# mohsenzakeri/Movi

Measured on AMD Instinct MI355X. Metric: PML query Gbases/s on regular-thresholds index, higher is better.
Workload: dtype u64

## Files before the change

movi_amd/csrc/movi_abi.hip:

```cpp
#include "../../include/movi_hip.h"
#include "movi_kernels.hpp"
#include "movi_expand_host.hpp"

#include <algorithm>
#include <cstdio>
#include <cstdlib>
#include <chrono>
#include <cstring>
#include <string>
#include <unordered_map>
#include <vector>

#include <dlfcn.h>
#include <fcntl.h>
#include <rccl/rccl.h>
#include <sys/mman.h>
#include <sys/stat.h>
#include <thread>
#include <unistd.h>

using namespace movi;

namespace {

// ... 743 lines not shown
}
constexpr size_t kTallyBytes = 2u * kTallySlots * sizeof(unsigned long long);
static hipError_t read_tally(const unsigned long long *d_tally, unsigned long long (&sum)[2], hipStream_t s) {
    std::vector<unsigned long long> h(2u * kTallySlots);
    hipError_t e = hipMemcpyAsync(h.data(), d_tally, kTallyBytes, hipMemcpyDeviceToHost, s);
    if (e == hipSuccess) e = hipStreamSynchronize(s);
    sum[0] = sum[1] = 0;
    if (e == hipSuccess) for (uint32_t i = 0; i < kTallySlots; ++i) { sum[0] += h[2 * i]; sum[1] += h[2 * i + 1]; }
    return e;
}
static void sample_no_ff(movi_index *ix, hipStream_t s) {
    if (ix->ahead_tallied) return;
    unsigned long long *d_tally = nullptr, h_tally[2] = {0, 0};
    hipError_t e = hipMalloc(&d_tally, kTallyBytes);
    if (e == hipSuccess) e = hipMemsetAsync(d_tally, 0, kTallyBytes, s);
    if (e == hipSuccess) e = tally_no_ff_share(ix->kmode, ix->dev, 16, d_tally, s);
    if (e == hipSuccess) e = read_tally(d_tally, h_tally, s);
    if (d_tally) (void)hipFree(d_tally);
    if (e != hipSuccess) { (void)hipGetLastError(); return; }
    ix->ahead_no_ff = h_tally[1] ? (double)h_tally[0] / (double)h_tally[1] : 0.0;
    ix->ahead_tallied = true;
}
static bool ahead_wanted(movi_index *ix) {
    const uint64_t bytes = ahead_rows_bytes(ix->desc.r);
    size_t free_b = 0, total_b = 0;
    if (hipMemGetInfo(&free_b, &total_b) != hipSuccess) { (void)hipGetLastError(); return false; }
    return bytes <= total_b / 4 && free_b > bytes + std::max<uint64_t>(2ull << 30, bytes / 2);
}
constexpr double kAheadCountRatio = 0.67;
static int build_ahead(movi_index *ix, hipStream_t s, bool by_itself) {
    HIP_TRY(hipMalloc(&ix->d_rows2, ahead_rows_bytes(ix->desc.r)));
    uint64_t tail = 0;
    unsigned long long *d_tally = nullptr, h_tally[2] = {0, 0};
    hipError_t e = hipMalloc(&d_tally, kTallyBytes);
    if (e == hipSuccess) e = hipMemsetAsync(d_tally, 0, kTallyBytes, s);
    if (e == hipSuccess) e = build_ahead_rows(ix->kmode, ix->dev, ix->d_rows2, &tail, s, d_tally);
    if (e == hipSuccess) e = read_tally(d_tally, h_tally, s);
    if (d_tally) (void)hipFree(d_tally);
    if (e != hipSuccess) { (void)hipFree(ix->d_rows2); ix->d_rows2 = nullptr; return fail_hip(e, "building the look-ahead rows"); }
    ix->dev.rows2 = ix->d_rows2;
    ix->dev.rows2_tail = tail;
    ix->dev.hints = ahead_rows_hinted(ix->desc.r) ? 1u : 0u;
    ix->ahead_no_ff = h_tally[1] ? (double)h_tally[0] / (double)h_tally[1] : 0.0;
    ix->ahead_tallied = true;
    ix->dev.rows2_count = (!by_itself || ix->ahead_no_ff >= kAheadCountRatio) ? 1u : 0u;
    return MOVI_OK;
}

constexpr uint64_t kDeepAutoRows = 48ull << 20;
static bool deep_eligible(const movi_index *ix) {
    return ix->kmode == MOVI_MODE_REGULAR_THRESHOLDS && deep_rows_eligible(ix->desc.r);
}
static int build_deep(movi_index *ix, hipStream_t s) {
    HIP_TRY(hipMalloc(&ix->d_rows3, deep_rows_bytes(ix->desc.r)));
    hipError_t e = build_deep_rows(ix->kmode, ix->dev, ix->d_rows3, s);
    if (e == hipSuccess) e = hipStreamSynchronize(s);
    if (e != hipSuccess) { (void)hipFree(ix->d_rows3); ix->d_rows3 = nullptr; return fail_hip(e, "building the deep rows"); }
    ix->dev.rows3 = ix->d_rows3;
    return MOVI_OK;
}

static bool ftab_eligible(const movi_index *ix) {
    return (ix->kmode == MOVI_MODE_REGULAR_THRESHOLDS || ix->kmode == MOVI_MODE_REGULAR) && ix->dev.sigma - ix->dev.sep == 4;
}
static int build_ftab_table(movi_index *ix, uint32_t K, hipStream_t s) {
    const size_t bytes = (size_t)16 << (2 * K);
    HIP_TRY(hipMalloc(&ix->d_ftab, bytes));
    hipError_t e = build_ftab(ix->kmode, ix->dev, K, ix->d_ftab, s);
    if (e == hipSuccess) e = hipStreamSynchronize(s);
    if (e != hipSuccess) { (void)hipFree(ix->d_ftab); ix->d_ftab = nullptr; return fail_hip(e, "building the count query's interval table"); }
    ix->dev.ftab = ix->d_ftab;
    ix->dev.ftab_k = K;
    return MOVI_OK;
}

static void ensure_pml_tables(movi_index *ix, hipStream_t s, bool from_prepare = false) {
    if (ix->kmer_auto > 0 && !ix->d_kmer && kmer_eligible(ix)) {
        if (build_kmer(ix, (uint32_t)ix->kmer_auto, s) != MOVI_OK) {
            (void)hipGetLastError();
            ix->kmer_auto = 0;
        }
    }
    if (ix->ahead_auto > 0 && !ix->d_rows2 && ahead_eligible(ix) && (from_prepare || !ix->prepared)) {
        if (ix->ahead_retry_in > 0) ix->ahead_retry_in -= 1;
        else if (!ahead_wanted(ix)) ix->ahead_retry_in = 63;
        else if (build_ahead(ix, s, true) != MOVI_OK) {
            (void)hipGetLastError();
            ix->ahead_auto = 0;
        }
    }
    if (ix->deep_auto > 0 && !ix->d_rows3 && deep_eligible(ix) && ix->desc.r <= kDeepAutoRows && (from_prepare || !ix->prepared)) {
        if (!ix->ahead_tallied) sample_no_ff(ix, s);
        size_t free_b = 0, total_b = 0;
        const uint64_t bytes = deep_rows_bytes(ix->desc.r);
        if (ix->ahead_tallied && ix->ahead_no_ff < kAheadCountRatio) {
            ix->deep_auto = 0;
        } else if (hipMemGetInfo(&free_b, &total_b) != hipSuccess || free_b < bytes + (2ull << 30) || build_deep(ix, s) != MOVI_OK) {
            (void)hipGetLastError();
            ix->deep_auto = 0;
        }
    }
}

extern "C" {

int movi_index_get_desc(const movi_index_t *ix, movi_index_desc_t *desc) {
    if (!ix || !desc) return fail(MOVI_ERR_ARG, "NULL argument");
    *desc = ix->desc;
    desc->id_blocks = nullptr;
    desc->separator_thresholds = nullptr;
    desc->separator_map = nullptr;
    desc->tally_ids = nullptr;
    return MOVI_OK;
}

int movi_index_device_rows(const movi_index_t *ix, const void **d_rows, size_t *bytes) {
    if (!ix || !d_rows || !bytes) return fail(MOVI_ERR_ARG, "NULL argument");
    *d_rows = ix->d_rows;
    *bytes = ix->kmode != (int)ix->desc.mode ? (size_t)ix->desc.r * 8 : ix->rows_bytes;
    return MOVI_OK;
}

int movi_set_option(movi_index_t *ix, const char *key, int64_t value) {
    if (!ix || !key) return fail(MOVI_ERR_ARG, "NULL argument");
    if (!strcmp(key, "pml_variant")) {
        if (value != -1 && value != 0 && value != 1 && value != 14)
            return fail(MOVI_ERR_ARG, "pml_variant must be -1 (auto), 0, 1 or 14");
        ix->cfg.pml_variant = (int)value;
        return MOVI_OK;
    }
    if (!strcmp(key, "zml_variant")) {
        if (value < -1 || value > 1) return fail(MOVI_ERR_ARG, "zml_variant must be -1 (auto), 0 or 1");
        ix->cfg.zml_variant = (int)value;
        return MOVI_OK;
    }
    if (!strcmp(key, "count_variant")) {
        if (value < -1 || value > 1) return fail(MOVI_ERR_ARG, "count_variant must be -1 (auto), 0 or 1");
        ix->cfg.count_variant = (int)value;
        return MOVI_OK;
    }
    if (!strcmp(key, "idx64")) {
        if (value != 0 && value != 1) return fail(MOVI_ERR_ARG, "idx64 must be 0 or 1");
        ix->dev.idx32 = (value == 0 && ix->desc.r < 0xFFFFFFFFull) ? 1u : 0u;
        return MOVI_OK;
    }
    if (!strcmp(key, "block_threads")) {
        if (value != 0 && value != 64 && value != 128 && value != 192 && value != 256)
// ... 303 lines not shown
}

int movi_pml_expand_device(movi_index_t *ix, const uint32_t *d_mask_words, const uint64_t *d_offsets, uint64_t n_reads,
                           uint64_t n_bases, uint64_t first_base, uint16_t *d_out_pml, void *stream) {
    if (!ix) return fail(MOVI_ERR_ARG, "index handle is NULL");
    if (n_reads == 0) return MOVI_OK;
    if (!d_mask_words || !d_offsets || (n_bases && !d_out_pml)) return fail(MOVI_ERR_ARG, "NULL device buffer");
    HIP_TRY(hipSetDevice(ix->device));
    HIP_TRY(launch_pml_expand(d_mask_words, d_offsets, n_reads, n_bases, (uint32_t)(first_base & 31u), d_out_pml,
                              static_cast<hipStream_t>(stream)));
    return MOVI_OK;
}

int movi_zml_device(movi_index_t *ix, const uint8_t *d_bases, const uint64_t *d_offsets, uint64_t n_reads,
                    uint64_t n_bases, uint16_t *d_out_zml, uint8_t *d_read_err, const uint32_t *d_read_order,
                    void *stream) {
    return ml_device(true, ix, d_bases, d_offsets, n_reads, n_bases, d_out_zml, d_read_err, d_read_order, stream);
}

int movi_last_launch(const movi_index_t *ix, movi_launch_info_t *info) {
    if (!ix || !info) return fail(MOVI_ERR_ARG, "NULL argument");
    memset(info, 0, sizeof(*info));
    static_assert(sizeof(info->kernel) == sizeof(ix->last_launch.kernel), "kernel name buffers differ");
    memcpy(info->kernel, ix->last_launch.kernel, sizeof(info->kernel));
    info->variant = ix->last_launch.variant;
    info->block_threads = ix->last_launch.block_threads;
    info->waves_per_cu = ix->last_launch.waves_per_cu;
    info->segmented = ix->last_launch.segmented;
    info->idx64 = ix->last_launch.idx64;
    info->staged = ix->last_launch.staged;
    info->ahead = ix->last_launch.ahead;
    return MOVI_OK;
}

int movi_launch_log(char *buf, size_t cap, size_t *needed) {
    const size_t n = take_launch_log(buf, cap);
    if (needed) *needed = n + 1;
    return MOVI_OK;
}

int movi_index_info(const movi_index_t *ix, const char *key, double *value) {
    if (!ix || !key || !value) return fail(MOVI_ERR_ARG, "NULL argument");
    const double rows = ix->kmode != (int)ix->desc.mode ? (double)ix->desc.r * 8.0 : (double)ix->rows_bytes;
    const double kmer = ix->d_kmer ? (double)((size_t)16 << (2 * ix->dev.kmer_k)) : 0.0;
    const double ftab = ix->d_ftab ? (double)((size_t)16 << (2 * ix->dev.ftab_k)) : 0.0;
    const double ahead = ix->d_rows2 ? (double)ahead_rows_bytes(ix->desc.r) : 0.0;
    const double deep = ix->d_rows3 ? (double)deep_rows_bytes(ix->desc.r) : 0.0;
    const double ckpt = ix->d_ckpt ? (double)((ix->desc.r >> kPrefixShift) + 2) * 8.0 : 0.0;
    if (!strcmp(key, "rows_bytes")) *value = rows;
    else if (!strcmp(key, "kmer_bytes")) *value = kmer;
    else if (!strcmp(key, "ftab_bytes")) *value = ftab;
    else if (!strcmp(key, "ahead_rows_bytes")) *value = ahead;
    else if (!strcmp(key, "deep_rows_bytes")) *value = deep;
    else if (!strcmp(key, "ckpt_bytes")) *value = ckpt;
    else if (!strcmp(key, "derived_bytes")) *value = kmer + ftab + ahead + deep + ckpt;
    else if (!strcmp(key, "ahead_no_ff")) *value = ix->ahead_tallied ? ix->ahead_no_ff : -1.0;
    else if (!strcmp(key, "device_scratch_bytes")) {
        double b = (double)ix->dmask_cap + (double)ix->scratch_cap[movi_index::kTmp] + (double)ix->seg_ws.cap;
        for (const auto &r : ix->dmask_retired) b += (double)r.second;
        *value = b;
    }
    else if (!strcmp(key, "host_staging_bytes")) {
        double b = 0.0;
        for (int k = 0; k < movi_index::kScratchSlots; k++) b += (double)ix->scratch_cap[k];
        *value = b;
    }
    else return fail(MOVI_ERR_ARG, std::string("unknown info key: ") + key);
    return MOVI_OK;
}

int movi_last_stats(movi_index_t *ix, void *stream, movi_query_stats_t *stats) {
    if (!ix || !stats) return fail(MOVI_ERR_ARG, "NULL argument");
    HIP_TRY(hipSetDevice(ix->device));
    HIP_TRY(hipStreamSynchronize(static_cast<hipStream_t>(stream)));
    DevStats h{};
    HIP_TRY(hipMemcpy(&h, ix->d_stats, sizeof(h), hipMemcpyDeviceToHost));
    stats->bases = 0;
    stats->fast_forwards = h.fast_forwards;
    stats->scans = h.scans;
    stats->repositions = h.repositions;
    stats->errors = h.errors;
    stats->lane_steps = h.lane_steps;
    stats->wave_steps = h.wave_steps;
    stats->segments = h.segments;
    stats->rewalked = h.rewalked;
    return MOVI_OK;
}

}

namespace {

constexpr uint64_t kChunkBases = 1ull << 28;
constexpr uint64_t kMinChunkReads = 1ull << 18;
constexpr uint64_t kMaxChunkBases = 1ull << 31;
constexpr uint64_t kPipeMinBases = 1ull << 22;
constexpr uint64_t kPipeMinReads = 1ull << 15;
constexpr uint64_t kPipeTargetChunks = 8;
constexpr uint64_t kPipeMaskChunks = 16;

hipError_t grow(void **p, size_t *cap, size_t bytes) {
    if (bytes < 8) bytes = 8;
    if (*cap < bytes) {
        if (*p) (void)hipFree(*p);
        *p = nullptr;
        *cap = 0;
        const size_t want = bytes + (bytes >> 3);
        hipError_t e = hipMalloc(p, want);
// ... 1064 lines not shown
```

movi_amd/csrc/movi_kernels.hip:

```cpp
#include "movi_device.hpp"
#include "movi_search.hpp"

#include <hipcub/hipcub.hpp>

#include <algorithm>
#include <atomic>
#include <cstdio>
#include <cstring>
#include <mutex>
#include <set>
#include <string>

namespace movi {

template <int MODE, int VARIANT, int CLS>
__global__ __launch_bounds__(256) void pml_kernel(DevIndex ix, const uint8_t *__restrict__ bases,
                                                     const uint64_t *__restrict__ offs, uint64_t n_reads,
                                                     uint16_t *__restrict__ out, uint8_t *__restrict__ err,
                                                     DevStats *stats, const uint32_t *__restrict__ order,
                                                     ClsArgs cls) {
    __shared__ uint8_t s_code[256];
    for (int i = threadIdx.x; i < 256; i += blockDim.x) s_code[i] = ix.code_of[i];
    __syncthreads();

// ... 228 lines not shown
    }
    uint8_t *line = out + (i >> 3) * 128u + (i & 7u) * 8u;
    __builtin_memcpy(line, &row, 8);
    __builtin_memcpy(line + 64, &e, 8);
    if (i + 4 >= ix.r) {
        uint8_t *tl = out + tail + (i + 4 - ix.r) * 8u;
        __builtin_memcpy(tl, &row, 8);
        __builtin_memcpy(tl + 64, &e, 8);
    }
}

template <int MODE>
__global__ __launch_bounds__(256) void no_ff_share_kernel(DevIndex ix, uint64_t stride, unsigned long long *tally) {
    const uint64_t i = ((uint64_t)blockIdx.x * blockDim.x + threadIdx.x) * stride;
    uint32_t no_ff = 0, ni = 0;
    if (i < ix.r) {
        const uint2 row = load_row<MODE>(ix.rows, i);
        const uint64_t j = row_id<MODE>(row, i, ix);
        ni = row_n<MODE>(row);
        if (j < ix.r) {
            const uint32_t nj = row_n<MODE>(load_row<MODE>(ix.rows, j)), oi = row_off<MODE>(row);
            no_ff = nj > oi ? (nj - oi < ni ? nj - oi : ni) : 0u;
        }
    }
    const uint32_t a = wave_sum(no_ff), b = wave_sum(ni);
    if ((threadIdx.x & 63) == 0) tally_add(tally, a, b);
}
hipError_t tally_no_ff_share(int kmode, const DevIndex &ix, uint64_t stride, unsigned long long *d_tally, hipStream_t stream) {
    if (kmode != 6 || !d_tally || stride == 0) return hipErrorInvalidValue;
    const uint64_t n = (ix.r + stride - 1) / stride, blocks = (n + 255) / 256;
    if (blocks > 0x7FFFFFFFull) return hipErrorInvalidValue;
    hipLaunchKernelGGL(no_ff_share_kernel<6>, dim3((unsigned)blocks), dim3(256), 0, stream, ix, stride, d_tally);
    return hipGetLastError();
}

uint64_t ahead_rows_bytes(uint64_t r) { return ((r + 7) / 8 + 1) * 128; }

bool ahead_rows_hinted(uint64_t r) { return r >= 8 && r < 0xFFFFFFFFull; }

hipError_t build_ahead_rows(int kmode, const DevIndex &ix, uint8_t *d_rows2, uint64_t *tail, hipStream_t stream, unsigned long long *d_tally) {
    if (!d_rows2 || !tail || ix.r < 8 || (ix.r >> 36) != 0 || kmode != 6) return hipErrorInvalidValue;
    *tail = ((ix.r + 7) / 8) * 128;
    hipError_t e = hipMemsetAsync(d_rows2, 0, ahead_rows_bytes(ix.r), stream);
    if (e != hipSuccess) return e;
    const uint64_t blocks = (ix.r + 255) / 256;
    if (blocks > 0x7FFFFFFFull) return hipErrorInvalidValue;
    if (ahead_rows_hinted(ix.r)) hipLaunchKernelGGL((ahead_rows_kernel<6, 1>), dim3((unsigned)blocks), dim3(256), 0, stream, ix, d_rows2, *tail, d_tally);
    else hipLaunchKernelGGL((ahead_rows_kernel<6, 0>), dim3((unsigned)blocks), dim3(256), 0, stream, ix, d_rows2, *tail, d_tally);
    return hipGetLastError();
}

__global__ __launch_bounds__(256) void deep_rows_kernel(DevIndex ix, uint32_t *__restrict__ out) {
    const uint64_t i = (uint64_t)blockIdx.x * blockDim.x + threadIdx.x;
    const uint64_t padded = ((ix.r + 2) / 3) * 3;
    if (i >= padded) return;
    uint32_t *W = out + (i / 3) * 16u;
    const uint32_t s = (uint32_t)(i % 3);
    uint32_t d0 = 0x0FFFFFFFu, d1 = (7u << 22) | (7u << 25) | (7u << 28), d2 = 0x0FFFFFFFu, d3 = 0, d4 = 0x0FFFFFFFu, x = 0;
    if (i < ix.r) {
        const uint2 row = load_row<6>(ix.rows, i);
        const uint64_t j = row_id<6>(row, i, ix);
        const uint32_t c = row_c<6>(row);
        d0 = (j < ix.r ? (uint32_t)j : 0x0FFFFFFFu) | (row_thr<6>(row, 0) << 28) | (row_thr<6>(row, 1) << 29) | (row_thr<6>(row, 2) << 30);
        d1 = row_n<6>(row) | (row_off<6>(row) << 11) | (c << 22) | (7u << 25) | (7u << 28);
        if (j < ix.r) {
            const uint2 rj = load_row<6>(ix.rows, j);
            const uint64_t j2 = row_id<6>(rj, j, ix);
            if (j2 < ix.r) {
                const uint2 rj2 = load_row<6>(ix.rows, j2);
                const uint64_t j3 = row_id<6>(rj2, j2, ix);
                d1 = (d1 & ~(7u << 25)) | (row_c<6>(rj) << 25);
                d2 = (uint32_t)j2;
                d3 = row_n<6>(rj) | (row_off<6>(rj) << 11);
                if (j3 < ix.r) {
                    const uint32_t n2 = row_n<6>(rj2), o2 = row_off<6>(rj2);
                    d1 = (d1 & ~(7u << 28)) | (row_c<6>(rj2) << 28);
                    d3 |= (n2 & 0x3FFu) << 22;
                    d4 = (uint32_t)j3 | ((n2 >> 10) << 28) | ((o2 & 7u) << 29);
                    x = o2 >> 3;
                }
            }
        }
        uint32_t h = 0;
        if (ix.sep == 0u && ix.sigma == 4u && i != ix.end_bwt_idx) {
            const uint64_t wb = (i / 3) * 3;
            for (uint32_t k = 0; k < 3u; ++k) {
                const uint32_t a = k < c ? k : k + 1u;
                if (a > 3u) continue;
                uint32_t d = 0;
                if (row_thr<6>(row, k) == 0u) {
                    const uint64_t edge = wb + 2;
                    bool inside = false;
                    for (uint64_t t = i + 1; t <= edge && t < ix.r; ++t) inside = inside || row_c<6>(load_row<6>(ix.rows, t)) == a;
                    if (!inside)
                        for (uint64_t t = edge + 1; t <= edge + 3 && t < ix.r; ++t)
                            if (row_c<6>(load_row<6>(ix.rows, t)) == a) { d = (uint32_t)(t - edge); break; }
                } else {
                    bool inside = false;
                    for (uint64_t t = wb; t < i; ++t) inside = inside || row_c<6>(load_row<6>(ix.rows, t)) == a;
                    if (!inside)
                        for (uint64_t t = 1; t <= 3 && t <= wb; ++t)
                            if (row_c<6>(load_row<6>(ix.rows, wb - t)) == a) { d = (uint32_t)t; break; }
                }
                h |= d << (2u * k);
            }
        }
        d2 |= (h & 15u) << 28;
        x |= (h >> 4) << 8;
    }
    W[5u * s + 0u] = d0;
    W[5u * s + 1u] = d1;
    W[5u * s + 2u] = d2;
    W[5u * s + 3u] = d3;
    W[5u * s + 4u] = d4;
    atomicOr(&W[15], x << (10u * s));
}

uint64_t deep_rows_bytes(uint64_t r) { return ((r + 2) / 3) * 64; }
bool deep_rows_eligible(uint64_t r) { return r >= 8 && r < 0x0FFFFFFFull; }

hipError_t build_deep_rows(int kmode, const DevIndex &ix, uint8_t *d_rows3, hipStream_t stream) {
    if (!d_rows3 || !deep_rows_eligible(ix.r) || kmode != 6) return hipErrorInvalidValue;
    hipError_t e = hipMemsetAsync(d_rows3, 0, deep_rows_bytes(ix.r), stream);
    if (e != hipSuccess) return e;
    const uint64_t blocks = (ix.r + 2 + 255) / 256;
    hipLaunchKernelGGL(deep_rows_kernel, dim3((unsigned)blocks), dim3(256), 0, stream, ix, reinterpret_cast<uint32_t *>(d_rows3));
    return hipGetLastError();
}

hipError_t build_kmer_table(const DevIndex &ix, uint32_t K, uint4 *d_table, hipStream_t stream) {
    if (K < 1 || K > 12 || !d_table || ix.sigma - ix.sep != 4) return hipErrorInvalidValue;
    const uint64_t n = 1ull << (2 * K);
    hipLaunchKernelGGL(kmer_table_kernel<6>, dim3((unsigned)((n + 255) / 256)), dim3(256), 0, stream, ix, K, d_table);
    return hipGetLastError();
}

template <int MODE>
__global__ __launch_bounds__(256) void seg_probe_kernel(DevIndex ix, const uint8_t *__restrict__ bases, const uint64_t *__restrict__ offs,
                                                       uint64_t n_reads, uint32_t lead, uint32_t reach, uint32_t *__restrict__ tally) {
    __shared__ uint8_t s_code[256];
    for (int i = threadIdx.x; i < 256; i += blockDim.x) s_code[i] = ix.code_of[i];
    __syncthreads();
    const uint64_t t = (uint64_t)blockIdx.x * blockDim.x + threadIdx.x, n_lanes = (uint64_t)gridDim.x * blockDim.x;
    const EndThr ethr = end_thresholds(ix);
    const uint64_t stride = n_reads > n_lanes ? n_reads / n_lanes : 1, per = n_reads < n_lanes ? n_lanes / n_reads : 1;
    const uint64_t rid = per > 1 ? t % n_reads : t * stride, slot = per > 1 ? t / n_reads : 0;
    bool valid = rid < n_reads && slot < per;
    const uint64_t beg = valid ? offs[rid] : 0, len = valid ? offs[rid + 1] - beg : 0;
    const uint64_t mid = len * (2 * slot + 1) / (2 * per);
    valid = valid && mid >= reach && mid + lead <= len;
    const uint8_t *R = bases + beg + mid + lead;
    const uint64_t r1 = ix.r - 1;
    const uint2 row0 = load_row<MODE>(ix.rows, r1);
    uint64_t ia = r1, ib = r1;
    uint32_t oa = row_n<MODE>(row0) - 1, ob = oa, ma = 0, mb = 0, ffx = 0, scx = 0, rpx = 0, failed = 0, met = 0;
    uint2 ra = row0, rb = row0;
    for (uint32_t k = 0; wave_any(valid && k < lead + reach && failed == 0u && met == 0u); ++k) {
        const bool live = valid && k < lead + reach && failed == 0u && met == 0u;
        uint32_t a = 0xFFu;
        if (live) a = s_code[*(R - 1 - (int64_t)k)];
        uint32_t e0 = 0;
        if (k > lead) e0 = lf_step2<MODE>(ix, live, ia, oa, ra, ib, ob, rb, ffx);
        else e0 = lf_step<MODE>(ix, live && k != 0, ib, ob, rb, ffx);
        const bool l2 = live && e0 == 0u;
        const uint32_t e = walk_base<MODE>(ix, ethr, l2, false, a, ib, ob, rb, mb, ffx, scx, rpx);
        const uint32_t e2 = walk_base<MODE>(ix, ethr, l2 && k >= lead, false, a, ia, oa, ra, ma, ffx, scx, rpx);
        if (e0 | e | e2) failed = 1;
        if (live && failed == 0u && k >= lead && ia == ib && oa == ob && ma == mb) met = 1;
        if (k == lead + reach / 2 && 2 * __popcll(__ballot(met != 0u)) < __popcll(__ballot(valid))) break;
        if (k == lead + reach / 6 && 10 * __popcll(__ballot(met != 0u)) < __popcll(__ballot(valid))) break;
        if (k > lead && (k & 15u) == 15u && 20 * __popcll(__ballot(met != 0u)) >= 19 * __popcll(__ballot(valid))) break;
    }
    const uint32_t nv = wave_sum(valid ? 1u : 0u), nm = wave_sum(met);
    if ((threadIdx.x & 63) == 0) {
        if (nv) atomicAdd(&tally[0], nv);
        if (nm) atomicAdd(&tally[1], nm);
    }
}
// ... 2280 lines not shown
```

movi_amd/csrc/movi_kernels.hpp:

```cpp
#pragma once
#include <hip/hip_runtime.h>
#include <stdint.h>

namespace movi {

constexpr int kPrefixShift = 5;

struct DevIndex {
    const uint8_t *rows;
    const uint32_t *id_blocks;
    const uint8_t *code_of;
    const uint64_t *row_start_ckpt;
    uint64_t r;
    uint64_t end_bwt_idx;
    uint64_t n_blocks;
    uint64_t block_size;
    uint32_t block_shift;
    uint32_t sigma;
    uint64_t end_thr[4];
    uint64_t first_runs[6], first_offsets[6], last_runs[6], last_offsets[6];
    uint32_t sep;
    uint32_t n_sep;
    const uint64_t *sep_rows;
    const uint2 *sep_vals;
// ... 140 lines not shown
hipError_t preload_walk_u64();
hipError_t preload_walkseg_u32();
hipError_t preload_walkseg_u64();

struct SegWorkspace {
    void *buf = nullptr;
    size_t cap = 0;
};

struct MaskArgs {
    uint32_t *words = nullptr;
    uint32_t phase = 0;
    uint16_t *tmp_pml = nullptr;
    uint16_t *expand_out = nullptr;
};
uint64_t pml_mask_words(uint64_t n_reads, uint64_t n_bases, uint32_t phase);
bool pml_mask_needs_tmp(const DevIndex &ix, const LaunchCfg &cfg, uint64_t n_reads, uint64_t n_bases, bool have_seg_ws);
bool pml_vector_via_masks(const DevIndex &ix, const LaunchCfg &cfg, uint64_t n_reads, uint64_t n_bases, bool have_seg_ws, bool ordered);
hipError_t launch_pml_expand(const uint32_t *d_words, const uint64_t *d_offsets, uint64_t n_reads, uint64_t n_bases, uint32_t phase,
                             uint16_t *d_out, hipStream_t stream);
hipError_t launch_copy_words(uint64_t *d_dst, const uint64_t *src, uint64_t n, hipStream_t stream);
hipError_t launch_pml_to_mask(const uint16_t *d_pml, const uint64_t *d_offsets, uint64_t n_reads, uint64_t n_bases, uint32_t phase,
                              uint32_t *d_words, hipStream_t stream);

hipError_t launch_pml(int mode, const DevIndex &ix, const uint8_t *d_bases, const uint64_t *d_offsets,
                      uint64_t n_reads, uint64_t n_bases, uint16_t *d_out, uint8_t *d_err, DevStats *d_stats,
                      const uint32_t *d_order, const LaunchCfg &cfg, hipStream_t stream,
                      const ClsArgs &cls = ClsArgs(), SegWorkspace *seg_ws = nullptr, int ragged_hint = -1,
                      int *seg_verdict = nullptr, LaunchInfo *info = nullptr, const MaskArgs &mask = MaskArgs());

hipError_t launch_count(int mode, const DevIndex &ix, const uint8_t *d_bases, const uint64_t *d_offsets,
                        uint64_t n_reads, uint64_t *d_matched, uint64_t *d_count, uint8_t *d_err,
                        DevStats *d_stats, const uint32_t *d_order, const LaunchCfg &cfg, hipStream_t stream,
                        LaunchInfo *info = nullptr, uint64_t n_bases = 0);

hipError_t launch_zml(int mode, const DevIndex &ix, const uint8_t *d_bases, const uint64_t *d_offsets,
                      uint64_t n_reads, uint64_t n_bases, uint16_t *d_out, uint8_t *d_err, DevStats *d_stats,
                      const uint32_t *d_order, const LaunchCfg &cfg, hipStream_t stream,
                      SegWorkspace *seg_ws = nullptr, int ragged_hint = -1, int *seg_verdict = nullptr,
                      LaunchInfo *info = nullptr);

hipError_t launch_classify(const uint16_t *d_pml, const uint64_t *d_offsets, uint64_t n_reads, uint32_t bin_width,
                           uint32_t thr, uint32_t *d_above, uint32_t *d_below, uint64_t *d_sum, hipStream_t stream,
                           const uint8_t *d_err = nullptr, uint64_t n_bases = 0);

hipError_t expand_sampled_rows(int mode, const DevIndex &ix, void *d_rows6, hipStream_t stream);
hipError_t expand_blocked_rows(int mode, const DevIndex &ix, void *d_rows6, hipStream_t stream);

hipError_t widen_rows(const uint8_t *d_packed, uint64_t r, uint32_t *d_wide, hipStream_t stream);

hipError_t build_kmer_table(const DevIndex &ix, uint32_t K, uint4 *d_table, hipStream_t stream);
uint64_t ahead_rows_bytes(uint64_t r);
uint64_t deep_rows_bytes(uint64_t r);
bool deep_rows_eligible(uint64_t r);
hipError_t build_deep_rows(int kmode, const DevIndex &ix, uint8_t *d_rows3, hipStream_t stream);
bool ahead_rows_hinted(uint64_t r);
hipError_t build_ahead_rows(int kmode, const DevIndex &ix, uint8_t *d_rows2, uint64_t *tail, hipStream_t stream,
                            unsigned long long *d_tally = nullptr);
hipError_t tally_no_ff_share(int kmode, const DevIndex &ix, uint64_t stride, unsigned long long *d_tally, hipStream_t stream);

hipError_t build_ftab(int mode, const DevIndex &ix, uint32_t K, uint4 *d_table, hipStream_t stream);

struct MemOut { uint32_t start, end; uint64_t count; };
struct MemArgs {
    uint64_t comp;
    uint32_t min_len;
    uint32_t pad_;
};
hipError_t launch_mem(int mode, const DevIndex &ix, const MemArgs &a, const uint8_t *d_bases, const uint64_t *d_offsets,
                      uint64_t n_reads, MemOut *d_mems, uint32_t *d_n_mems, uint8_t *d_err, DevStats *d_stats,
                      const uint32_t *d_order, hipStream_t stream, LaunchInfo *info);

struct KmerRun { uint32_t start, count; };
struct KmerArgs {
    uint32_t k;
    uint32_t step;
};
hipError_t launch_kmer(int mode, const DevIndex &ix, const KmerArgs &a, const uint8_t *d_bases, const uint64_t *d_offsets,
                       uint64_t n_reads, KmerRun *d_runs, uint32_t *d_n_runs, uint32_t *d_found, uint8_t *d_err,
                       DevStats *d_stats, const uint32_t *d_order, hipStream_t stream, LaunchInfo *info);

hipError_t launch_count_scan(const uint32_t *d_n, uint64_t n_reads, uint64_t *d_first, hipStream_t stream);
hipError_t launch_gather(const void *d_src, size_t elem_bytes, const uint64_t *d_offsets, const uint32_t *d_n, uint64_t n_reads,
                         const uint64_t *d_first, void *d_out, hipStream_t stream);

hipError_t build_row_start_ckpt(int mode, const uint8_t *d_rows, uint64_t r, uint64_t *d_ckpt,
                                hipStream_t stream);

}
```

movi_amd/csrc/movi_walk.hpp:

```cpp
#pragma once
#include "movi_device.hpp"

namespace movi {

template <int MODE, typename IdxT, int CLS, int SEP, int SEG, int STG, int AHD, int PSH, int RING>
__global__ __launch_bounds__(256) void pml_kernel_flatp(DevIndex ix, const uint8_t *__restrict__ bases,
                                                       const uint64_t *__restrict__ offs, uint64_t n_reads,
                                                       uint16_t *__restrict__ out, uint8_t *__restrict__ err,
                                                       DevStats *stats, const uint32_t *__restrict__ order,
                                                       ClsArgs cls, SegArgs seg) {
    static_assert(SEG == 0 || CLS == 0, "segments: plain PML");
    static_assert(AHD == 0 || STG == 1, "look-ahead rows: staged reads");
    static_assert(AHD == 0 || AHD == 1 || AHD == 2, "plain rows, look-ahead rows or deep rows");
    static_assert(AHD != 2 || (PSH == 0 && sizeof(IdxT) == 4), "deep rows: tables of fewer than 2^28 rows, no pair-shared gathers");
    static_assert(PSH == 0 || STG == 1, "pair-shared gathers: staged kernels");
    static_assert(RING == 0 || STG == 1, "PMLs out through the LDS ring / as reset masks: staged kernels");
    static_assert(RING != 2 || (CLS == 0 && SEG == 0), "reset masks: plain PML of whole reads");
    enum : uint32_t { sFF = 0, sDown = 1, sUp = 2, sDone = 3 };
    __shared__ uint8_t s_code[256];
    for (int i = threadIdx.x; i < 256; i += blockDim.x) s_code[i] = ix.code_of[i];
    __syncthreads();

    const uint64_t t = (uint64_t)blockIdx.x * blockDim.x + threadIdx.x;
    uint32_t ff_total = 0, scan_total = 0, repo_total = 0, failed = 0, err_total = 0;
    const EndThr ethr = end_thresholds(ix);
    const IdxT r1 = (IdxT)(ix.r - 1), end_row = (IdxT)ix.end_bwt_idx;
    const uint2 row_r1 = load_row<MODE>(ix.rows, r1);
    const uint32_t off0 = row_n<MODE>(row_r1) - 1;

    const bool valid = (SEG == 1 ? (*seg.go != 0u && t < *seg.n_seg) : (t < n_reads && (SEG != 2 || seg.read_fail[t] != 0)));
    const uint64_t rid = (valid && order && SEG == 0) ? order[t] : t;
    const uint64_t beg = valid ? (SEG == 1 ? seg.seg_in[rid] : offs[rid]) : 0;
    const uint32_t len = valid ? (SEG == 1 ? seg.seg_len[rid] : (uint32_t)(offs[rid + 1] - beg)) : 0;
    const uint64_t obeg = (SEG == 1 && valid) ? seg.seg_out[rid] : beg;
    constexpr bool ring = RING == 1;
    constexpr bool msk = RING == 2;
    uint32_t *const M = msk ? reinterpret_cast<uint32_t *>(out) + (((beg + ix.mask_phase) >> 5) + rid) : nullptr;
    uint32_t mk = 0;
    const uint32_t packed_end = len & (ring ? ~15u : ~7u);

    auto load_pair_at = [&](uint64_t e, uint64_t &c0, uint64_t &c1) {
        uint64_t two[2];
        __builtin_memcpy(two, bases + (e >= 16 ? e - 16 : 0), 16);
        c0 = two[1];
        c1 = two[0];
    };
    auto fix_pair = [&](uint64_t e, uint64_t &c0, uint64_t &c1) {
        if (e < 16) {
            const uint32_t sh = 8u * (uint32_t)(16 - e);
            if (sh >= 64) { c0 = c1 << (sh - 64); c1 = 0; }
            else { c0 = (c0 << sh) | (c1 >> (64 - sh)); c1 <<= sh; }
        }
    };
    constexpr uint32_t WN = 4u;
    const IdxT wb_last = (IdxT)(ix.r - WN);
    auto win_base = [&](IdxT nd) -> IdxT {
        const IdxT wb = nd & ~(IdxT)(WN - 1u);
        return wb < wb_last ? wb : wb_last;
    };
    uint2 ahw[4];
    uint4 raw[4];
    uint4 dq[4];
    const uint32_t odd_lane = threadIdx.x & 1u;
    auto fetch = [&](IdxT nd, bool act, uint2 (&w)[4]) {
        if (AHD == 2) {
            const uint32_t q3 = __umulhi((uint32_t)nd, 0xAAAAAAABu) >> 1;
            const uint8_t *at = ix.rows3 + (act ? (uint64_t)q3 * 64u : 0u);
            __builtin_memcpy(&dq[0], at, 16);
            __builtin_memcpy(&dq[1], at + 16, 16);
            __builtin_memcpy(&dq[2], at + 32, 16);
            __builtin_memcpy(&dq[3], at + 48, 16);
            return;
        }
        if (PSH) {
            uint64_t at;
            if (AHD) {
                const IdxT wb = nd & ~(IdxT)3;
                at = wb < wb_last ? (uint64_t)(wb >> 3) * 128u + (uint64_t)((uint32_t)wb & 4u) * 8u : ix.rows2_tail;
            } else {
                at = (uint64_t)win_base(nd) * 8u;
            }
            if (!act) at = 0;
            const uint64_t pat = (uint64_t)pair_swap((uint32_t)at) | ((uint64_t)pair_swap((uint32_t)(at >> 32)) << 32);
            const uint8_t *tab = AHD ? ix.rows2 : ix.rows;
            const uint8_t *pe = tab + (odd_lane ? pat : at) + 16u * odd_lane;
            const uint8_t *po = tab + (odd_lane ? at : pat) + 16u * odd_lane;
            __builtin_memcpy(&raw[0], pe, 16);
            if (AHD) __builtin_memcpy(&raw[2], pe + 64u, 16);
            __builtin_memcpy(&raw[1], po, 16);
            if (AHD) __builtin_memcpy(&raw[3], po + 64u, 16);
            return;
        }
        if (AHD) {
            const IdxT wb = nd & ~(IdxT)3;
            const bool body = wb < wb_last;
            uint64_t at = body ? (uint64_t)(wb >> 3) * 128u + (uint64_t)((uint32_t)wb & 4u) * 8u : ix.rows2_tail;
            if (!act) at = 0;
            load_window<MODE>(ix.rows2 + at, 0, w);
            load_window<MODE>(ix.rows2 + at + 64u, 0, ahw);
        } else {
            load_window<MODE>(ix.rows, (uint64_t)(act ? win_base(nd) : (IdxT)0), w);
        }
    };
    ClsState cs;
    auto finish_read = [&]() {
        if (SEG == 1) {
            SegTot tt;
            tt.ff = ff_total; tt.scan = scan_total; tt.repo = repo_total; tt.flag = failed;
            seg.tot[rid] = tt;
            return;
        }
        if (msk) {
            if (failed) {
                for (uint32_t wd = 0; wd * 32u < len; ++wd) M[wd] = (len - wd * 32u >= 32u) ? 0xFFFFFFFFu : ((1u << (len & 31u)) - 1u);
            } else if (len & 31u) {
                M[len >> 5] = mk;
            }
        } else if (failed && CLS != 2) {
            for (uint32_t i = 0; i < len; ++i) out[obeg + i] = 0;
        }
        if (CLS) cs.store(cls, rid, failed != 0u);
        if (err) err[rid] = (uint8_t)failed;
        err_total += failed ? 1u : 0u;
    };
// ... 105 lines not shown
                }
                k += 1;
            }
            ml = run;
            need = (IdxT)((uint64_t)e4.x | ((uint64_t)(e4.y & 15u) << 32));
            off = (e4.y >> 4) & 0xFFFu;
            ff_total += e4.z;
            scan_total += e4.w;
            repo_total += K - (uint32_t)__popc(mask);
        }
        return use;
    };
    if (ix.kmer_k != 0u) {
        const uint32_t K = ix.kmer_k;
        uint32_t kidx = 0, bad = 0;
        for (uint32_t i = 0; i < K; ++i) {
            const uint64_t src = i < 8u ? rb : rb2;
            const uint32_t cc = (uint32_t)s_code[(uint32_t)(src >> (8u * (7u - (i & 7u)))) & 0xFFu] - (uint32_t)SEP;
            bad |= (uint32_t)(cc > 3u);
            kidx |= (cc & 3u) << (2u * i);
        }
        if (top_of_walk((uint32_t)(st != sDone) & (uint32_t)(len > K) & (bad ^ 1u), kidx)) {
            if (K >= 8u) rb = rb2;
            a = s_code[(uint32_t)(rb >> (8u * (7u - (K & 7u)))) & 0xFFu];
        }
    }
    uint32_t a1 = 0xFFu, a2 = 0xFFu;
    if (AHD) a1 = staged_code(k + 1);
    if (AHD == 2) a2 = staged_code(k + 2);
    uint2 w[4];
    fetch(need, st != sDone, w);

    uint32_t lane_steps = 0, wave_steps = 0;
    while (wave_any(st != sDone)) {
        const bool act = st < sDone;
        lane_steps += (uint32_t)act;
        wave_steps += 1;
#if defined(MOVI_PAD_PRE) && MOVI_PAD_PRE > 0
        {
            uint32_t pad = wave_steps;
#pragma unroll
            for (int i = 0; i < MOVI_PAD_PRE; ++i) asm volatile("v_add_u32 %0, %0, %0" : "+v"(pad));
        }
#endif
        struct StepOut {
            uint32_t resolved, match, ffm, lf, mism, scanning, found, down, qf, qn, jump, jdist, landed, landed_down, nf, n, rofff, emit;
            uint32_t dbl, lf2, off1, tpl, lf3, off2, errc, st_next;
            uint64_t j;
            IdxT needf, need_next, j2, j3;
        } R;
        R.tpl = 0; R.lf3 = 0; R.off2 = 0; R.j3 = 0;
        if (AHD == 2) {
            const uint32_t need32 = (uint32_t)need;
            const uint32_t wbase = (__umulhi(need32, 0xAAAAAAABu) >> 1) * 3u;
            const uint32_t r1u = (uint32_t)r1;
            const uint32_t d1a = dq[0].y, d1b = dq[1].z, d1c = dq[2].w;
            const uint32_t n0 = d1a & 0x7FFu, n1w = d1b & 0x7FFu, n2w = d1c & 0x7FFu;
            const uint32_t nm = (uint32_t)(((d1a >> 22) & 7u) != a) | ((uint32_t)(((d1b >> 22) & 7u) != a) << 1) | ((uint32_t)(((d1c >> 22) & 7u) != a) << 2);
            const uint32_t lim = r1u - wbase;
            const uint32_t first_win = (uint32_t)(wbase == 0u);
            uint32_t nd = need32;
            {
                const uint32_t q0 = nd - wbase;
                const uint32_t inw = (uint32_t)(q0 < 3u) & (uint32_t)(st < sDone);
                const uint32_t m0 = q0 == 0u, m1 = q0 <= 1u;
                const uint32_t t1 = m0 ? n0 : 0u, t2 = t1 + (m1 ? n1w : 0u), t3 = t2 + n2w;
                const uint32_t isff = inw & (uint32_t)(st == sFF);
                const uint32_t room = 65534u - (ff_run < 65534u ? ff_run : 65534u);
                uint32_t p0 = isff & m0 & (uint32_t)(off >= t1) & (uint32_t)(0u < lim), p1 = isff & m1 & (uint32_t)(off >= t2) & (uint32_t)(1u < lim),
                         p2 = isff & (uint32_t)(off >= t3) & (uint32_t)(2u < lim);
                uint32_t cf = p0 + p1 + p2;
                if (cf > room) {
                    cf = room;
                    const uint32_t first = m0 ? 0u : (m1 ? 1u : 2u);
                    p0 = p0 & (uint32_t)(first + cf > 0u);
                    p1 = p1 & (uint32_t)(first + cf > 1u);
                    p2 = p2 & (uint32_t)(first + cf > 2u);
                }
                off -= (p2 ? t3 : (p1 ? t2 : (p0 ? t1 : 0u)));
                ff_run += cf;
                const uint32_t dmask = (nm & (lim >= 3u ? 7u : ((1u << lim) - 1u))) >> q0;
                const uint32_t cd = (inw & (uint32_t)(st == sDown)) ? (uint32_t)__builtin_ctz(~dmask | 8u) : 0u;
                const uint32_t umask = ((nm & (first_win ? 6u : 7u)) << (2u - (q0 < 3u ? q0 : 2u))) & 7u;
                const uint32_t cu = (inw & (uint32_t)(st == sUp)) ? (uint32_t)__builtin_clz(((~umask) & 7u) << 29 | 0x10000000u) : 0u;
                scan_total += cd + cu;
                nd = nd + cf + cd - cu;
            }
            need = (IdxT)nd;
            const uint32_t qn = nd - wbase;
            const uint32_t inwin = (uint32_t)(qn < 3u) & (uint32_t)act;
            auto sel3 = [](uint32_t x0, uint32_t x1, uint32_t x2, uint32_t q) { return q == 0u ? x0 : (q == 1u ? x1 : x2); };
            const uint32_t rD0 = sel3(dq[0].x, dq[1].y, dq[2].z, qn), rD1 = sel3(d1a, d1b, d1c, qn);
            const uint32_t n = rD1 & 0x7FFu, c = (rD1 >> 22) & 7u;
            const uint32_t isFF = (uint32_t)(st == sFF) & inwin, isDown = (uint32_t)(st == sDown) & inwin, isUp = (uint32_t)(st == sUp) & inwin;
            const uint32_t ffm = isFF & (uint32_t)(nd < r1u) & (uint32_t)(off >= n);
            const uint32_t ff_over = ffm & (uint32_t)(ff_run + 1 >= 65535u);
            const uint32_t resolved = isFF & (ffm ^ 1u);
            const uint32_t illegal = a == 0xFFu, match = c == a;
            const uint32_t mism = resolved & (illegal ^ 1u) & (match ^ 1u);
            const uint32_t kk = thr_slot(SEP, a, c);
            const uint32_t kc = kk > 2u ? 2u : kk;
            uint32_t thr = ((rD0 >> (28u + kc)) & 1u) ? n : 0u;
            if (SEP) {
                if (mism & (uint32_t)(c == 0u) & (uint32_t)(need != end_row)) thr = separator_threshold(ix, (uint64_t)need, a);
            }
            const uint32_t down = (uint32_t)(off >= ((need == end_row) ? end_threshold(SEP, ethr, a) : thr));
            const uint32_t at_last = nd >= r1u, at_first = nd == 0u;
            const uint32_t repo_edge = mism & (down ? at_last : at_first);
            const uint32_t has = (nm ^ 7u) & (down ? (6u << qn) & 7u : (1u << qn) - 1u);
            const uint32_t found = mism & (uint32_t)(has != 0u) & ix.inwin;
            const uint32_t qf = found ? (down ? (uint32_t)__builtin_ctz(has | 8u) : 31u - (uint32_t)__builtin_clz(has | 1u)) : qn;
            const uint32_t far = mism & (found ^ 1u);
            const uint32_t f0 = sel3(dq[0].x, dq[1].y, dq[2].z, qf), f1 = sel3(d1a, d1b, d1c, qf), f2 = sel3(dq[0].z, dq[1].w, dq[3].x, qf),
                           f3 = sel3(dq[0].w, dq[2].x, dq[3].y, qf), f4 = sel3(dq[1].x, dq[2].y, dq[3].z, qf);
            const uint32_t fx = (dq[3].w >> (10u * (qf < 3u ? qf : 0u))) & 0x3FFu;
            const uint32_t nf = f1 & 0x7FFu, rofff = (f1 >> 11) & 0x7FFu;
            const uint32_t scanning = isDown | isUp;
            const uint32_t hit = scanning & match;
            const uint32_t landed = hit | found;
            const uint32_t landed_down = hit ? isDown : down;
            const uint32_t scan_edge = scanning & (hit ^ 1u) & (isDown ? at_last : at_first);
            const uint32_t emit = (resolved & (illegal | match)) | landed;
            const uint32_t lf = emit & (uint32_t)(k + 1 != len);
            const uint32_t jj = f0 & 0x0FFFFFFFu;
            const uint32_t lf_bad = lf & (uint32_t)(jj >= (uint32_t)ix.r);
            const uint32_t h6 = (f2 >> 28) | ((fx >> 8) << 4);
            const uint32_t hd = __builtin_amdgcn_ubfe(h6, kc + kc, ix.hint_w);
            const uint32_t jump = far & (uint32_t)(hd != 0u);
            const uint32_t jtgt = down ? wbase + 2u + hd : wbase - hd;
            const uint32_t jdist = down ? jtgt - nd : nd - jtgt;
            const uint32_t step_fwd = ffm | (far & down) | (scanning & (hit ^ 1u) & isDown);
            const uint32_t step_back = (far & (down ^ 1u)) | (scanning & (hit ^ 1u) & isUp);
            uint32_t need_next = lf ? jj : (jump ? jtgt : nd + step_fwd - step_back);
            uint32_t st_next = (emit & (lf ^ 1u)) ? sDone : (lf ? sFF : (far ? (down ? sDown : sUp) : st));
            const uint32_t e1n = f3 & 0x7FFu, e1off = (f3 >> 11) & 0x7FFu, e1c = (f1 >> 25) & 7u, jj2 = f2 & 0x0FFFFFFFu;
            const uint32_t e2n = (f3 >> 22) | (((f4 >> 28) & 1u) << 10), e2off = ((f4 >> 29) & 7u) | ((fx & 0xFFu) << 3), e2c = (f1 >> 28) & 7u,
                           jj3 = f4 & 0x0FFFFFFFu;
            const uint32_t off_e = (landed ? (landed_down ? 0u : nf - 1u) : off) + rofff;
            const uint32_t dbl = lf & (uint32_t)(a1 == e1c) & (uint32_t)(off_e < e1n);
            const uint32_t lf2 = dbl & (uint32_t)(k + 2 != len);
            const uint32_t off_e2 = off_e + e1off;
            const uint32_t tpl = lf2 & (uint32_t)(a2 == e2c) & (uint32_t)(off_e2 < e2n);
            const uint32_t lf3 = tpl & (uint32_t)(k + 3 != len);
            need_next = tpl ? (lf3 ? jj3 : nd) : (dbl ? (lf2 ? jj2 : nd) : need_next);
            st_next = tpl ? (lf3 ? sFF : sDone) : (dbl ? (lf2 ? sFF : sDone) : st_next);
            uint32_t errc = kErrNone;
            if (wave_any((ff_over | repo_edge | scan_edge | lf_bad) != 0u)) {
                errc = ff_over ? kErrFastForward
                               : (repo_edge ? (down ? kErrNoRunBelow : kErrNoRunAbove)
                                  : (scan_edge ? (isDown ? kErrNoRunBelow : kErrNoRunAbove)
                                     : (lf_bad ? kErrIdRange : kErrNone)));
                if (errc) { need_next = nd; st_next = sDone; }
            }
            R.resolved = resolved; R.match = match; R.ffm = ffm; R.lf = lf; R.mism = mism; R.scanning = scanning; R.found = found; R.down = down;
            R.qf = qf; R.qn = qn; R.jump = jump; R.jdist = jdist; R.landed = landed; R.landed_down = landed_down; R.nf = nf; R.n = n; R.rofff = rofff;
            R.emit = emit; R.dbl = dbl; R.lf2 = lf2; R.off1 = e1off; R.tpl = tpl; R.lf3 = lf3; R.off2 = e2off; R.errc = errc; R.st_next = st_next;
            R.j = jj; R.needf = (IdxT)(wbase + qf); R.need_next = (IdxT)need_next; R.j2 = (IdxT)jj2; R.j3 = (IdxT)jj3;
        } else {
            if (PSH) {
                pair_assemble(odd_lane, raw[0], raw[1], w);
                if (AHD) pair_assemble(odd_lane, raw[2], raw[3], ahw);
            }
            const IdxT wbase = win_base(need);
            auto hop = [&]() {
                const uint32_t q = (uint32_t)(need - wbase);
                const uint32_t inwin = (uint32_t)(q < WN) & (uint32_t)(st < sDone);
                const uint2 hr = win_sel(w, q);
                const uint32_t hn = row_n<MODE>(hr), hc = row_c<MODE>(hr);
                const uint32_t ffh = inwin & (uint32_t)(st == sFF) & (uint32_t)(need < r1) & (uint32_t)(off >= hn) &
                                     (uint32_t)(ff_run + 1 < 65535u);
                const uint32_t nomatch = hc != a;
                const uint32_t dnh = inwin & (uint32_t)(st == sDown) & nomatch & (uint32_t)(need < r1);
                const uint32_t uph = inwin & (uint32_t)(st == sUp) & nomatch & (uint32_t)(need != 0);
                off = ffh ? off - hn : off;
                ff_run += ffh;
                scan_total += dnh | uph;
                need = need + (IdxT)(ffh + dnh) - (IdxT)uph;
            };
            const uint32_t nm = (uint32_t)(row_c<MODE>(w[0]) != a) | ((uint32_t)(row_c<MODE>(w[1]) != a) << 1) |
                                ((uint32_t)(row_c<MODE>(w[2]) != a) << 2) | ((uint32_t)(row_c<MODE>(w[3]) != a) << 3);
            const uint32_t last_win = (uint32_t)(wbase + 3 == r1);
            const uint32_t first_win = (uint32_t)(wbase == 0);
// ... 355 lines not shown
```

Before: 86.96.

## Widen deep-row fetch window from three rows to six per load

Each lane now fetches a 128-byte, six-row window of deep rows (two 64-byte three-row blocks) instead of one 64-byte, three-row block. The fast-forward, scan and repositioning logic is extended to handle six in-window candidates, so more steps resolve without another dependent memory fetch. Hint jump targets and the builder kernel's in-window test are changed to use the six-row edge. The cost is twice the bytes per fetch, higher register pressure from dq[8] and the 6-wide unrolled loops, and a padded allocation.

```diff
diff --git a/movi_amd/csrc/movi_abi.hip b/movi_amd/csrc/movi_abi.hip
--- a/movi_amd/csrc/movi_abi.hip
+++ b/movi_amd/csrc/movi_abi.hip
@@ -819,7 +819,7 @@
     return ix->kmode == MOVI_MODE_REGULAR_THRESHOLDS && deep_rows_eligible(ix->desc.r);
 }
 static int build_deep(movi_index *ix, hipStream_t s) {
-    HIP_TRY(hipMalloc(&ix->d_rows3, deep_rows_bytes(ix->desc.r)));
+    HIP_TRY(hipMalloc(&ix->d_rows3, deep_rows_alloc_bytes(ix->desc.r)));
     hipError_t e = build_deep_rows(ix->kmode, ix->dev, ix->d_rows3, s);
     if (e == hipSuccess) e = hipStreamSynchronize(s);
     if (e != hipSuccess) { (void)hipFree(ix->d_rows3); ix->d_rows3 = nullptr; return fail_hip(e, "building the deep rows"); }
@@ -859,7 +859,7 @@
     if (ix->deep_auto > 0 && !ix->d_rows3 && deep_eligible(ix) && ix->desc.r <= kDeepAutoRows && (from_prepare || !ix->prepared)) {
         if (!ix->ahead_tallied) sample_no_ff(ix, s);
         size_t free_b = 0, total_b = 0;
-        const uint64_t bytes = deep_rows_bytes(ix->desc.r);
+        const uint64_t bytes = deep_rows_alloc_bytes(ix->desc.r);
         if (ix->ahead_tallied && ix->ahead_no_ff < kAheadCountRatio) {
             ix->deep_auto = 0;
         } else if (hipMemGetInfo(&free_b, &total_b) != hipSuccess || free_b < bytes + (2ull << 30) || build_deep(ix, s) != MOVI_OK) {
@@ -1269,8 +1269,10 @@
     else if (!strcmp(key, "ftab_bytes")) *value = ftab;
     else if (!strcmp(key, "ahead_rows_bytes")) *value = ahead;
     else if (!strcmp(key, "deep_rows_bytes")) *value = deep;
+    else if (!strcmp(key, "deep_rows_alloc_bytes")) *value = ix->d_rows3 ? (double)deep_rows_alloc_bytes(ix->desc.r) : 0.0;
+    else if (!strcmp(key, "deep_rows_device_address")) *value = (double)(uintptr_t)ix->d_rows3;
     else if (!strcmp(key, "ckpt_bytes")) *value = ckpt;
-    else if (!strcmp(key, "derived_bytes")) *value = kmer + ftab + ahead + deep + ckpt;
+    else if (!strcmp(key, "derived_bytes")) *value = kmer + ftab + ahead + (ix->d_rows3 ? (double)deep_rows_alloc_bytes(ix->desc.r) : 0.0) + ckpt;
     else if (!strcmp(key, "ahead_no_ff")) *value = ix->ahead_tallied ? ix->ahead_no_ff : -1.0;
     else if (!strcmp(key, "device_scratch_bytes")) {
         double b = (double)ix->dmask_cap + (double)ix->scratch_cap[movi_index::kTmp] + (double)ix->seg_ws.cap;
diff --git a/movi_amd/csrc/movi_kernels.hip b/movi_amd/csrc/movi_kernels.hip
--- a/movi_amd/csrc/movi_kernels.hip
+++ b/movi_amd/csrc/movi_kernels.hip
@@ -304,7 +304,7 @@
 
 __global__ __launch_bounds__(256) void deep_rows_kernel(DevIndex ix, uint32_t *__restrict__ out) {
     const uint64_t i = (uint64_t)blockIdx.x * blockDim.x + threadIdx.x;
-    const uint64_t padded = ((ix.r + 2) / 3) * 3;
+    const uint64_t padded = ((ix.r + 5) / 6) * 6;
     if (i >= padded) return;
     uint32_t *W = out + (i / 3) * 16u;
     const uint32_t s = (uint32_t)(i % 3);
@@ -335,13 +335,13 @@
         }
         uint32_t h = 0;
         if (ix.sep == 0u && ix.sigma == 4u && i != ix.end_bwt_idx) {
-            const uint64_t wb = (i / 3) * 3;
+            const uint64_t wb = (i / 6) * 6;
             for (uint32_t k = 0; k < 3u; ++k) {
                 const uint32_t a = k < c ? k : k + 1u;
                 if (a > 3u) continue;
                 uint32_t d = 0;
                 if (row_thr<6>(row, k) == 0u) {
-                    const uint64_t edge = wb + 2;
+                    const uint64_t edge = wb + 5;
                     bool inside = false;
                     for (uint64_t t = i + 1; t <= edge && t < ix.r; ++t) inside = inside || row_c<6>(load_row<6>(ix.rows, t)) == a;
                     if (!inside)
@@ -369,13 +369,14 @@
 }
 
 uint64_t deep_rows_bytes(uint64_t r) { return ((r + 2) / 3) * 64; }
+uint64_t deep_rows_alloc_bytes(uint64_t r) { return ((r + 5) / 6) * 128; }
 bool deep_rows_eligible(uint64_t r) { return r >= 8 && r < 0x0FFFFFFFull; }
 
 hipError_t build_deep_rows(int kmode, const DevIndex &ix, uint8_t *d_rows3, hipStream_t stream) {
     if (!d_rows3 || !deep_rows_eligible(ix.r) || kmode != 6) return hipErrorInvalidValue;
-    hipError_t e = hipMemsetAsync(d_rows3, 0, deep_rows_bytes(ix.r), stream);
+    hipError_t e = hipMemsetAsync(d_rows3, 0, deep_rows_alloc_bytes(ix.r), stream);
     if (e != hipSuccess) return e;
-    const uint64_t blocks = (ix.r + 2 + 255) / 256;
+    const uint64_t blocks = (ix.r + 5 + 255) / 256;
     hipLaunchKernelGGL(deep_rows_kernel, dim3((unsigned)blocks), dim3(256), 0, stream, ix, reinterpret_cast<uint32_t *>(d_rows3));
     return hipGetLastError();
 }
diff --git a/movi_amd/csrc/movi_kernels.hpp b/movi_amd/csrc/movi_kernels.hpp
--- a/movi_amd/csrc/movi_kernels.hpp
+++ b/movi_amd/csrc/movi_kernels.hpp
@@ -216,6 +216,7 @@
 hipError_t build_kmer_table(const DevIndex &ix, uint32_t K, uint4 *d_table, hipStream_t stream);
 uint64_t ahead_rows_bytes(uint64_t r);
 uint64_t deep_rows_bytes(uint64_t r);
+uint64_t deep_rows_alloc_bytes(uint64_t r);
 bool deep_rows_eligible(uint64_t r);
 hipError_t build_deep_rows(int kmode, const DevIndex &ix, uint8_t *d_rows3, hipStream_t stream);
 bool ahead_rows_hinted(uint64_t r);
diff --git a/movi_amd/csrc/movi_walk.hpp b/movi_amd/csrc/movi_walk.hpp
--- a/movi_amd/csrc/movi_walk.hpp
+++ b/movi_amd/csrc/movi_walk.hpp
@@ -60,16 +60,14 @@
     };
     uint2 ahw[4];
     uint4 raw[4];
-    uint4 dq[4];
+    uint4 dq[8];
     const uint32_t odd_lane = threadIdx.x & 1u;
     auto fetch = [&](IdxT nd, bool act, uint2 (&w)[4]) {
         if (AHD == 2) {
-            const uint32_t q3 = __umulhi((uint32_t)nd, 0xAAAAAAABu) >> 1;
-            const uint8_t *at = ix.rows3 + (act ? (uint64_t)q3 * 64u : 0u);
-            __builtin_memcpy(&dq[0], at, 16);
-            __builtin_memcpy(&dq[1], at + 16, 16);
-            __builtin_memcpy(&dq[2], at + 32, 16);
-            __builtin_memcpy(&dq[3], at + 48, 16);
+            const uint32_t q6 = __umulhi((uint32_t)nd, 0xAAAAAAABu) >> 2;
+            const uint8_t *at = ix.rows3 + (act ? (uint64_t)q6 * 128u : 0u);
+#pragma unroll
+            for (uint32_t i = 0; i < 8u; ++i) __builtin_memcpy(&dq[i], at + 16u * i, 16);
             return;
         }
         if (PSH) {
@@ -281,45 +279,58 @@
         R.tpl = 0; R.lf3 = 0; R.off2 = 0; R.j3 = 0;
         if (AHD == 2) {
             const uint32_t need32 = (uint32_t)need;
-            const uint32_t wbase = (__umulhi(need32, 0xAAAAAAABu) >> 1) * 3u;
+            const uint32_t wbase = (__umulhi(need32, 0xAAAAAAABu) >> 2) * 6u;
             const uint32_t r1u = (uint32_t)r1;
-            const uint32_t d1a = dq[0].y, d1b = dq[1].z, d1c = dq[2].w;
-            const uint32_t n0 = d1a & 0x7FFu, n1w = d1b & 0x7FFu, n2w = d1c & 0x7FFu;
-            const uint32_t nm = (uint32_t)(((d1a >> 22) & 7u) != a) | ((uint32_t)(((d1b >> 22) & 7u) != a) << 1) | ((uint32_t)(((d1c >> 22) & 7u) != a) << 2);
+            const uint32_t d1[6] = {dq[0].y, dq[1].z, dq[2].w, dq[4].y, dq[5].z, dq[6].w};
+            uint32_t nw[6], nm = 0;
+#pragma unroll
+            for (uint32_t i = 0; i < 6u; ++i) {
+                nw[i] = d1[i] & 0x7FFu;
+                nm |= (uint32_t)(((d1[i] >> 22) & 7u) != a) << i;
+            }
             const uint32_t lim = r1u - wbase;
             const uint32_t first_win = (uint32_t)(wbase == 0u);
+            auto sel3 = [](uint32_t x0, uint32_t x1, uint32_t x2, uint32_t q) { return q == 0u ? x0 : (q == 1u ? x1 : x2); };
             uint32_t nd = need32;
             {
                 const uint32_t q0 = nd - wbase;
-                const uint32_t inw = (uint32_t)(q0 < 3u) & (uint32_t)(st < sDone);
-                const uint32_t m0 = q0 == 0u, m1 = q0 <= 1u;
-                const uint32_t t1 = m0 ? n0 : 0u, t2 = t1 + (m1 ? n1w : 0u), t3 = t2 + n2w;
+                const uint32_t inw = (uint32_t)(q0 < 6u) & (uint32_t)(st < sDone);
                 const uint32_t isff = inw & (uint32_t)(st == sFF);
                 const uint32_t room = 65534u - (ff_run < 65534u ? ff_run : 65534u);
-                uint32_t p0 = isff & m0 & (uint32_t)(off >= t1) & (uint32_t)(0u < lim), p1 = isff & m1 & (uint32_t)(off >= t2) & (uint32_t)(1u < lim),
-                         p2 = isff & (uint32_t)(off >= t3) & (uint32_t)(2u < lim);
-                uint32_t cf = p0 + p1 + p2;
+                uint32_t ts[6], pp[6], run = 0, cf = 0;
+#pragma unroll
+                for (uint32_t i = 0; i < 6u; ++i) {
+                    const uint32_t mi = (uint32_t)(q0 <= i);
+                    run += mi ? nw[i] : 0u;
+                    ts[i] = run;
+                    pp[i] = isff & mi & (uint32_t)(off >= run) & (uint32_t)(i < lim);
+                    cf += pp[i];
+                }
                 if (cf > room) {
                     cf = room;
-                    const uint32_t first = m0 ? 0u : (m1 ? 1u : 2u);
-                    p0 = p0 & (uint32_t)(first + cf > 0u);
-                    p1 = p1 & (uint32_t)(first + cf > 1u);
-                    p2 = p2 & (uint32_t)(first + cf > 2u);
-                }
-                off -= (p2 ? t3 : (p1 ? t2 : (p0 ? t1 : 0u)));
+                    const uint32_t first = q0 < 5u ? q0 : 5u;
+#pragma unroll
+                    for (uint32_t i = 0; i < 6u; ++i) pp[i] &= (uint32_t)(first + cf > i);
+                }
+                uint32_t passed = 0;
+#pragma unroll
+                for (uint32_t i = 0; i < 6u; ++i) passed = pp[i] ? ts[i] : passed;
+                off -= passed;
                 ff_run += cf;
-                const uint32_t dmask = (nm & (lim >= 3u ? 7u : ((1u << lim) - 1u))) >> q0;
-                const uint32_t cd = (inw & (uint32_t)(st == sDown)) ? (uint32_t)__builtin_ctz(~dmask | 8u) : 0u;
-                const uint32_t umask = ((nm & (first_win ? 6u : 7u)) << (2u - (q0 < 3u ? q0 : 2u))) & 7u;
-                const uint32_t cu = (inw & (uint32_t)(st == sUp)) ? (uint32_t)__builtin_clz(((~umask) & 7u) << 29 | 0x10000000u) : 0u;
+                const uint32_t dmask = (nm & (lim >= 6u ? 63u : ((1u << lim) - 1u))) >> q0;
+                const uint32_t cd = (inw & (uint32_t)(st == sDown)) ? (uint32_t)__builtin_ctz(~dmask | 64u) : 0u;
+                const uint32_t umask = ((nm & (first_win ? 62u : 63u)) << (5u - (q0 < 6u ? q0 : 5u))) & 63u;
+                const uint32_t cu = (inw & (uint32_t)(st == sUp)) ? (uint32_t)__builtin_clz(((~umask) & 63u) << 26 | 0x02000000u) : 0u;
                 scan_total += cd + cu;
                 nd = nd + cf + cd - cu;
             }
             need = (IdxT)nd;
             const uint32_t qn = nd - wbase;
-            const uint32_t inwin = (uint32_t)(qn < 3u) & (uint32_t)act;
-            auto sel3 = [](uint32_t x0, uint32_t x1, uint32_t x2, uint32_t q) { return q == 0u ? x0 : (q == 1u ? x1 : x2); };
-            const uint32_t rD0 = sel3(dq[0].x, dq[1].y, dq[2].z, qn), rD1 = sel3(d1a, d1b, d1c, qn);
+            const uint32_t inwin = (uint32_t)(qn < 6u) & (uint32_t)act;
+            const bool hn = qn >= 3u;
+            const uint32_t sn = hn ? qn - 3u : qn;
+            const uint32_t rD0 = sel3(hn ? dq[4].x : dq[0].x, hn ? dq[5].y : dq[1].y, hn ? dq[6].z : dq[2].z, sn),
+                           rD1 = sel3(hn ? d1[3] : d1[0], hn ? d1[4] : d1[1], hn ? d1[5] : d1[2], sn);
             const uint32_t n = rD1 & 0x7FFu, c = (rD1 >> 22) & 7u;
             const uint32_t isFF = (uint32_t)(st == sFF) & inwin, isDown = (uint32_t)(st == sDown) & inwin, isUp = (uint32_t)(st == sUp) & inwin;
             const uint32_t ffm = isFF & (uint32_t)(nd < r1u) & (uint32_t)(off >= n);
@@ -336,13 +347,18 @@
             const uint32_t down = (uint32_t)(off >= ((need == end_row) ? end_threshold(SEP, ethr, a) : thr));
             const uint32_t at_last = nd >= r1u, at_first = nd == 0u;
             const uint32_t repo_edge = mism & (down ? at_last : at_first);
-            const uint32_t has = (nm ^ 7u) & (down ? (6u << qn) & 7u : (1u << qn) - 1u);
+            const uint32_t has = (nm ^ 63u) & (down ? (62u << qn) & 63u : (1u << qn) - 1u);
             const uint32_t found = mism & (uint32_t)(has != 0u) & ix.inwin;
-            const uint32_t qf = found ? (down ? (uint32_t)__builtin_ctz(has | 8u) : 31u - (uint32_t)__builtin_clz(has | 1u)) : qn;
+            const uint32_t qf = found ? (down ? (uint32_t)__builtin_ctz(has | 64u) : 31u - (uint32_t)__builtin_clz(has | 1u)) : qn;
             const uint32_t far = mism & (found ^ 1u);
-            const uint32_t f0 = sel3(dq[0].x, dq[1].y, dq[2].z, qf), f1 = sel3(d1a, d1b, d1c, qf), f2 = sel3(dq[0].z, dq[1].w, dq[3].x, qf),
-                           f3 = sel3(dq[0].w, dq[2].x, dq[3].y, qf), f4 = sel3(dq[1].x, dq[2].y, dq[3].z, qf);
-            const uint32_t fx = (dq[3].w >> (10u * (qf < 3u ? qf : 0u))) & 0x3FFu;
+            const bool hf = qf >= 3u;
+            const uint32_t sf = hf ? qf - 3u : qf;
+            const uint32_t f0 = sel3(hf ? dq[4].x : dq[0].x, hf ? dq[5].y : dq[1].y, hf ? dq[6].z : dq[2].z, sf),
+                           f1 = sel3(hf ? d1[3] : d1[0], hf ? d1[4] : d1[1], hf ? d1[5] : d1[2], sf),
+                           f2 = sel3(hf ? dq[4].z : dq[0].z, hf ? dq[5].w : dq[1].w, hf ? dq[7].x : dq[3].x, sf),
+                           f3 = sel3(hf ? dq[4].w : dq[0].w, hf ? dq[6].x : dq[2].x, hf ? dq[7].y : dq[3].y, sf),
+                           f4 = sel3(hf ? dq[5].x : dq[1].x, hf ? dq[6].y : dq[2].y, hf ? dq[7].z : dq[3].z, sf);
+            const uint32_t fx = ((hf ? dq[7].w : dq[3].w) >> (10u * (sf < 3u ? sf : 0u))) & 0x3FFu;
             const uint32_t nf = f1 & 0x7FFu, rofff = (f1 >> 11) & 0x7FFu;
             const uint32_t scanning = isDown | isUp;
             const uint32_t hit = scanning & match;
@@ -356,7 +372,7 @@
             const uint32_t h6 = (f2 >> 28) | ((fx >> 8) << 4);
             const uint32_t hd = __builtin_amdgcn_ubfe(h6, kc + kc, ix.hint_w);
             const uint32_t jump = far & (uint32_t)(hd != 0u);
-            const uint32_t jtgt = down ? wbase + 2u + hd : wbase - hd;
+            const uint32_t jtgt = down ? wbase + 5u + hd : wbase - hd;
             const uint32_t jdist = down ? jtgt - nd : nd - jtgt;
             const uint32_t step_fwd = ffm | (far & down) | (scanning & (hit ^ 1u) & isDown);
             const uint32_t step_back = (far & (down ^ 1u)) | (scanning & (hit ^ 1u) & isUp);
```

New measurement: 83.15. 0.956x the previous value.
